# ClashLuke/LocAtE

Measured on AMD Instinct MI355X. Metric: images/sec (G+D step) 64x64 bs=64, higher is better.
Workload: dtype f32 (contractions fp32-faithful on the matrix cores: 2 x scaled fp16 operand pieces / 3 MFMAs per slice where the operand's largest magnitude comes with it, else 3 x bf16 pieces / 6 MFMAs; fp32 accumulate); 1 GPU; LocAtE G+D step, 64x64 RGB, batch 64 per GPU (the fp32 variant - the reference's own precision - of BASELINE.json configs[1]: 64x64 RGB bs 64), self/feature attention at 16x16 and 64x64, random-init weights; global_batch=64, image_size=64, parallelism=dp1, launch=hipGraph replay, G-step generator pass on a second stream

## Files before the change

include/locate_hip.h:

```cpp
#ifndef LOCATE_HIP_H
#define LOCATE_HIP_H
#include <stddef.h>
#include <stdint.h>
#ifdef __cplusplus
extern "C" {
#endif

const char* locate_last_error(void);
int locate_abi_version(void);
int locate_device_info(char* arch_name, int name_len, int* cu_count, int* wave_size);

int locate_roottanh_fwd(const float* x, float* y, int64_t n, void* absmax , void* stream);
int locate_absmax_words(void);
int locate_roottanh_bwd(const float* x, const float* gy, float* gx, int64_t n, int accumulate, void* absmax, void* stream);
int locate_absmax(const float* x, int64_t n, void* absmax, void* stream);
int locate_act_cat_rows_fwd(const float* latent, const float* pre, float* out, int rows, int z, int w, void* stream);
int locate_act_rows_bwd(const float* pre, const float* g, int64_t g_row_stride, const float* g_add, float* gpre, int rows, int w,
                        void* stream);
int locate_add3(const float* a, int64_t a_bs, const float* b, int64_t b_bs, const float* c, int64_t c_bs, float* out, int batch,
                int64_t per, void* stream);
int locate_tanh_fwd(const float* x, float* y, int64_t n, void* stream);
int locate_tanh_bwd(const float* y, const float* gy, float* gx, int64_t n, void* stream);

size_t locate_norm_stats_workspace_bytes(void);
// ... 12 lines not shown
                          void* workspace, int accumulate_dx, void* stream);
int locate_fin_norm_channels(const void* records, int n, void* stream);
size_t locate_channel_sum_workspace_bytes(int B, int C, int hw);
int locate_channel_sum(const float* g, float* out, int B, int C, int hw, int64_t batch_stride, void* workspace, void* stream);

int locate_gate_fwd(const float* x, const float* a, int a_per_plane, const float* gamma, float* out, int64_t planes, int hw,
                    void* stream);
int locate_gate_fwd_stats(const float* x, const float* a, int a_per_plane, const float* gamma, float* out, int64_t planes,
                          int hw, int groups, double* stats_partial, void* stream);
size_t locate_gate_bwd_workspace_bytes(int64_t planes);
int locate_gate_bwd_partials(int64_t planes, int hw);
int locate_gate_bwd(const float* x, const float* a, int a_per_plane, const float* gamma, const float* g, float* dx, float* da,
                    float* dgamma, int64_t planes, int hw, void* workspace, int accumulate_dx,
                    void* da_absmax , void* stream);

int locate_softmax_fwd(const float* x, float* y, int64_t rows, int n, void* stream);
int locate_softmax_bwd(const float* y, const float* gy, float* gx, int64_t rows, int n, void* stream);

int locate_upsample2x_fwd(const float* x, float* y, int64_t planes, int H, int W, void* stream);
int locate_upsample2x_bwd(const float* gy, float* gx, int64_t planes, int H, int W, void* stream);
int locate_pool2_upsample2x_fwd(const float* x, float* y, int64_t planes, int H, int W, void* stream);
int locate_pool2_upsample2x_bwd(const float* gy, float* gx, int64_t planes, int H, int W, int accumulate, void* stream);
int locate_avgpool2_fwd(const float* x, float* y, int64_t planes, int H, int W, void* stream);
int locate_avgpool2_bwd(const float* gy, float* gx, int64_t planes, int H, int W, int accumulate, void* stream);
int locate_feature_pool_fwd(const float* x, float* y, int64_t n_out, int r, void* stream);
int locate_feature_pool_bwd(const float* gy, float* gx, int64_t n_out, int r, int accumulate, void* stream);
int locate_copy_channels(const float* src, float* dst, int B, int C, int hw, int64_t src_batch_stride,
                         int64_t dst_batch_stride, int accumulate, void* stream);

size_t locate_sn_workspace_bytes(int h, int wd);
int locate_sn_power_iter(const float* w, float* u, float* v, float* sigma, float* wv, int h, int wd, void* workspace,
                         void* stream);
size_t locate_sn_table_record_bytes(void);
int locate_sn_power_iter_batched(const void* table, int n_layers, int max_h, int max_wd, void* stream);
int locate_sn_weight_bwd(const double* inner_partial, int n_partial, const float* u, const float* v, const float* sigma,
                         const float* wv, float* gw, float* du, float* dsigma_out, int h, int wd, void* stream);
size_t locate_sn_group_workspace_bytes(void);
int locate_sn_weight_bwd_grouped(const float* gy, int64_t gy_bs, const float* y, int64_t y_bs, const float* bias, int groups,
                                 int Bg, int M, int plane, const float* sigma_tab, int sigma_stride, const float* u,
                                 const float* v, const float* wv, int64_t wv_stride, float* gw, float* du,
                                 float* dsigma_total_out, int h, int wd, void* workspace, void* stream);
int locate_sn_dv_batched(const void* table, int n_layers, int max_h, int max_wd, void* stream);

size_t locate_conv_panel_bytes(const int* geom, int adjoint);
int locate_conv_pack_panel(const int* geom, int adjoint, const float* w, float* panel, void* stream);
size_t locate_conv_pack_job_bytes(void);
int locate_conv_pack_job(const int* geom, int adjoint, const float* w, float* panel, int block_start, void* job_out,
                         int* blocks_out, int direct, const void* weight_absmax);
int locate_conv_pack_panels(const void* jobs, int n_jobs, int total_blocks, int any_f16, int passes, void* stream);
int locate_conv_pack_job_is_direct(const void* job);
int locate_conv_pack_job_is_window(const void* job);
int locate_conv_win_ok(const int* geom, int adjoint_fmt, int64_t x_bs, const void* x);
size_t locate_conv_win_workspace_bytes(const int* geom, int adjoint_fmt);
size_t locate_conv_fwd_workspace_bytes(const int* geom);
size_t locate_conv_counter_bytes(void);
int locate_conv_fwd(const int* geom, const float* x, int64_t x_bs, const float* panel, const float* scale,
                    int scale_group_batch, int scale_stride, const float* bias, float* y, int64_t y_bs, void* workspace,
                    void* counters, int precision, const void* x_absmax, const void* act_epilogue, void* stream);
size_t locate_conv_dgrad_workspace_bytes(const int* geom);
int locate_conv_dgrad(const int* geom, const float* gy, int64_t gy_bs, const float* panel, const float* scale,
                      int scale_group_batch, int scale_stride, const float* bias, float* gx, int64_t gx_bs, void* workspace,
                      void* counters, int precision, const void* gy_absmax, const void* act_epilogue, void* stream);
size_t locate_conv_wgrad_workspace_bytes(const int* geom);
int locate_conv_wgrad_partials(const int* geom);
int locate_conv_wgrad(const int* geom, const float* x, int64_t x_bs, const float* gy, int64_t gy_bs, float* gw,
                      const float* w_ref, const float* inv_scale, int scale_group_batch, int scale_stride,
                      double* inner_partial, void* workspace, int precision, const void* x_absmax, const void* gy_absmax,
                      void* deferred_reduce, void* stream);
int locate_conv_wgrad_group_partials(const int* geom, int groups);
size_t locate_conv_wgrad_group_workspace_bytes(const int* geom, int groups);
size_t locate_slab_reduce_record_bytes(void);
int locate_slab_reduce_max(void);
int locate_slab_reduce_record_blocks(const void* record);
int locate_slab_reduce_batch(const void* records, int n, void* stream);

size_t locate_wgrad_batch_record_bytes(void);
int locate_wgrad_batch_max(void);
int locate_wgrad_batch_record(const int* geom, const float* x, int64_t x_bs, const float* gy, int64_t gy_bs, float* gw,
                              const float* w_ref, const float* inv_scale, int scale_group_batch, int scale_stride,
                              double* inner_partial, void* record);
int locate_wgrad_batch(const void* records, int n, void* stream);

int locate_dwconv_fwd(const int* geom, const float* x, int64_t x_bs, const float* w, const float* scale, int scale_group_batch,
                      int scale_stride, float* y, int64_t y_bs, void* stream);
int locate_dwconv_dgrad(const int* geom, const float* gy, int64_t gy_bs, const float* w, const float* scale,
                        int scale_group_batch, int scale_stride, float* gx, int64_t gx_bs, void* stream);
size_t locate_dwconv_wgrad_workspace_bytes(const int* geom);
int locate_dwconv_wgrad_partials(const int* geom);
int locate_dwconv_wgrad(const int* geom, const float* big, int64_t big_bs, const float* small, int64_t small_bs, float* gw,
                        const float* w_ref, const float* inv_scale, int scale_group_batch, int scale_stride,
                        double* inner_partial, void* workspace, void* stream);
int locate_groupdot_fwd(const float* x, int64_t x_bs, const float* w, const float* scale, int scale_group_batch,
                        int scale_stride, float* y, int B, int G, int L, void* stream);
int locate_groupdot_dgrad(const float* gy, const float* w, const float* scale, int scale_group_batch, int scale_stride,
                          float* gx, int64_t gx_bs, int B, int G, int L, void* stream);
int locate_groupdot_wgrad_partials(int G, int L);
int locate_groupdot_wgrad(const float* x, int64_t x_bs, const float* gy, float* gw, const float* w_ref, const float* inv_scale,
                          int scale_group_batch, int scale_stride, double* inner_partial, int B, int G, int L, void* stream);

size_t locate_fin_record_bytes(void);
int locate_fin_sn_dot_partials(int Bg, int M, int plane);
int locate_fin_sn_dots(const void* records, int n, void* stream);
int locate_fin_sn_rank1(const void* records, int n, void* stream);
int locate_fin_sums(const void* records, int n, void* stream);
int locate_fin_channel_slices(int B, int C, int hw);
int locate_fin_channel_sums(const void* records, int n, void* stream);
// ... 69 lines not shown
```

locate_amd/_lib.py:

```python
import ctypes
import os

import torch

_HERE = os.path.dirname(os.path.abspath(__file__))
LIB_PATH = os.path.join(_HERE, "csrc", "liblocate_hip_dbg.so" if os.environ.get("LOCATE_HIP_DEBUG_LIBRARY") == "1"
                        else "liblocate_hip.so")

c_p = ctypes.c_void_p
c_i = ctypes.c_int
c_i64 = ctypes.c_int64
c_f = ctypes.c_float
c_d = ctypes.c_double
c_sz = ctypes.c_size_t
c_ip = ctypes.POINTER(ctypes.c_int)

PROTOTYPES = {
    "locate_last_error": (ctypes.c_char_p, []),
    "locate_abi_version": (c_i, []),
    "locate_device_info": (c_i, [ctypes.c_char_p, c_i, c_ip, c_ip]),
    "locate_roottanh_fwd": (c_i, [c_p, c_p, c_i64, c_p, c_p]),
    "locate_roottanh_bwd": (c_i, [c_p, c_p, c_p, c_i64, c_i, c_p, c_p]),
    "locate_act_cat_rows_fwd": (c_i, [c_p, c_p, c_p, c_i, c_i, c_i, c_p]),
    "locate_act_rows_bwd": (c_i, [c_p, c_p, c_i64, c_p, c_p, c_i, c_i, c_p]),
    "locate_add3": (c_i, [c_p, c_i64, c_p, c_i64, c_p, c_i64, c_p, c_i, c_i64, c_p]),
    "locate_absmax_words": (c_i, []),
    "locate_wgrad_batch_record_bytes": (c_sz, []),
    "locate_wgrad_batch_max": (c_i, []),
    "locate_wgrad_batch_record": (c_i, [c_ip, c_p, c_i64, c_p, c_i64, c_p, c_p, c_p, c_i, c_i, c_p, c_p]),
    "locate_wgrad_batch": (c_i, [c_p, c_i, c_p]),
    "locate_absmax": (c_i, [c_p, c_i64, c_p, c_p]),
    "locate_tanh_fwd": (c_i, [c_p, c_p, c_i64, c_p]),
    "locate_tanh_bwd": (c_i, [c_p, c_p, c_p, c_i64, c_p]),
    "locate_norm_stats_workspace_bytes": (c_sz, []),
    "locate_norm_stats": (c_i, [c_p, c_i64, c_p, c_p, c_p]),
    "locate_norm_bwd_workspace_bytes": (c_sz, [c_i, c_i]),
    "locate_norm_fwd": (c_i, [c_p, c_p, c_i, c_p, c_p, c_i, c_p, c_i, c_i, c_i, c_i, c_p, c_p, c_p, c_p]),
    "locate_norm_bwd": (c_i, [c_p, c_p, c_p, c_p, c_i, c_p, c_i, c_p, c_p, c_p, c_i, c_i, c_i, c_i, c_p, c_i, c_p]),
    "locate_norm_bwd_fused_workspace_bytes": (c_sz, [c_i, c_i]),
    "locate_norm_bwd_fused_plane_offset": (c_sz, []),
    "locate_norm_bwd_fused": (c_i, [c_p, c_p, c_p, c_p, c_i, c_p, c_i, c_p, c_p, c_i, c_i, c_i, c_i, c_p, c_i, c_p]),
    "locate_fin_norm_channels": (c_i, [c_p, c_i, c_p]),
    "locate_channel_sum_workspace_bytes": (c_sz, [c_i, c_i, c_i]),
    "locate_channel_sum": (c_i, [c_p, c_p, c_i, c_i, c_i, c_i64, c_p, c_p]),
    "locate_gate_fwd": (c_i, [c_p, c_p, c_i, c_p, c_p, c_i64, c_i, c_p]),
    "locate_gate_fwd_stats": (c_i, [c_p, c_p, c_i, c_p, c_p, c_i64, c_i, c_i, c_p, c_p]),
    "locate_gate_bwd_workspace_bytes": (c_sz, [c_i64]),
    "locate_gate_bwd": (c_i, [c_p, c_p, c_i, c_p, c_p, c_p, c_p, c_p, c_i64, c_i, c_p, c_i, c_p, c_p]),
    "locate_softmax_fwd": (c_i, [c_p, c_p, c_i64, c_i, c_p]),
    "locate_softmax_bwd": (c_i, [c_p, c_p, c_p, c_i64, c_i, c_p]),
    "locate_upsample2x_fwd": (c_i, [c_p, c_p, c_i64, c_i, c_i, c_p]),
    "locate_upsample2x_bwd": (c_i, [c_p, c_p, c_i64, c_i, c_i, c_p]),
    "locate_pool2_upsample2x_fwd": (c_i, [c_p, c_p, c_i64, c_i, c_i, c_p]),
    "locate_pool2_upsample2x_bwd": (c_i, [c_p, c_p, c_i64, c_i, c_i, c_i, c_p]),
    "locate_avgpool2_fwd": (c_i, [c_p, c_p, c_i64, c_i, c_i, c_p]),
    "locate_avgpool2_bwd": (c_i, [c_p, c_p, c_i64, c_i, c_i, c_i, c_p]),
    "locate_feature_pool_fwd": (c_i, [c_p, c_p, c_i64, c_i, c_p]),
    "locate_feature_pool_bwd": (c_i, [c_p, c_p, c_i64, c_i, c_i, c_p]),
    "locate_copy_channels": (c_i, [c_p, c_p, c_i, c_i, c_i, c_i64, c_i64, c_i, c_p]),
    "locate_sn_workspace_bytes": (c_sz, [c_i, c_i]),
    "locate_sn_power_iter": (c_i, [c_p, c_p, c_p, c_p, c_p, c_i, c_i, c_p, c_p]),
    "locate_sn_table_record_bytes": (c_sz, []),
    "locate_sn_power_iter_batched": (c_i, [c_p, c_i, c_i, c_i, c_p]),
    "locate_sn_weight_bwd": (c_i, [c_p, c_i, c_p, c_p, c_p, c_p, c_p, c_p, c_p, c_i, c_i, c_p]),
    "locate_sn_group_workspace_bytes": (c_sz, []),
    "locate_sn_weight_bwd_grouped": (c_i, [c_p, c_i64, c_p, c_i64, c_p, c_i, c_i, c_i, c_i, c_p, c_i, c_p, c_p, c_p, c_i64, c_p,
                                           c_p, c_p, c_i, c_i, c_p, c_p]),
    "locate_sn_dv_batched": (c_i, [c_p, c_i, c_i, c_i, c_p]),
    "locate_conv_panel_bytes": (c_sz, [c_ip, c_i]),
    "locate_conv_pack_panel": (c_i, [c_ip, c_i, c_p, c_p, c_p]),
    "locate_conv_pack_job_bytes": (c_sz, []),
    "locate_conv_pack_job": (c_i, [c_ip, c_i, c_p, c_p, c_i, c_p, c_ip, c_i, c_p]),
    "locate_conv_pack_panels": (c_i, [c_p, c_i, c_i, c_i, c_i, c_p]),
    "locate_conv_pack_job_is_direct": (c_i, [c_p]),
    "locate_conv_pack_job_is_window": (c_i, [c_p]),
    "locate_conv_win_ok": (c_i, [c_ip, c_i, c_i64, c_p]),
    "locate_conv_win_workspace_bytes": (c_sz, [c_ip, c_i]),
    "locate_conv_fwd_workspace_bytes": (c_sz, [c_ip]),
    "locate_conv_counter_bytes": (c_sz, []),
    "locate_conv_fwd": (c_i, [c_ip, c_p, c_i64, c_p, c_p, c_i, c_i, c_p, c_p, c_i64, c_p, c_p, c_i, c_p, c_p, c_p]),
    "locate_conv_dgrad_workspace_bytes": (c_sz, [c_ip]),
    "locate_conv_dgrad": (c_i, [c_ip, c_p, c_i64, c_p, c_p, c_i, c_i, c_p, c_p, c_i64, c_p, c_p, c_i, c_p, c_p, c_p]),
    "locate_conv_wgrad_workspace_bytes": (c_sz, [c_ip]),
    "locate_conv_wgrad_partials": (c_i, [c_ip]),
    "locate_conv_wgrad": (c_i, [c_ip, c_p, c_i64, c_p, c_i64, c_p, c_p, c_p, c_i, c_i, c_p, c_p, c_i, c_p, c_p, c_p, c_p]),
    "locate_conv_wgrad_group_partials": (c_i, [c_ip, c_i]),
    "locate_conv_wgrad_group_workspace_bytes": (c_sz, [c_ip, c_i]),
    "locate_slab_reduce_record_bytes": (c_sz, []),
    "locate_slab_reduce_max": (c_i, []),
    "locate_slab_reduce_record_blocks": (c_i, [c_p]),
    "locate_slab_reduce_batch": (c_i, [c_p, c_i, c_p]),
    "locate_dwconv_fwd": (c_i, [c_ip, c_p, c_i64, c_p, c_p, c_i, c_i, c_p, c_i64, c_p]),
    "locate_dwconv_dgrad": (c_i, [c_ip, c_p, c_i64, c_p, c_p, c_i, c_i, c_p, c_i64, c_p]),
    "locate_dwconv_wgrad_workspace_bytes": (c_sz, [c_ip]),
    "locate_dwconv_wgrad_partials": (c_i, [c_ip]),
    "locate_dwconv_wgrad": (c_i, [c_ip, c_p, c_i64, c_p, c_i64, c_p, c_p, c_p, c_i, c_i, c_p, c_p, c_p]),
    "locate_groupdot_fwd": (c_i, [c_p, c_i64, c_p, c_p, c_i, c_i, c_p, c_i, c_i, c_i, c_p]),
    "locate_groupdot_dgrad": (c_i, [c_p, c_p, c_p, c_i, c_i, c_p, c_i64, c_i, c_i, c_i, c_p]),
    "locate_groupdot_wgrad_partials": (c_i, [c_i, c_i]),
    "locate_groupdot_wgrad": (c_i, [c_p, c_i64, c_p, c_p, c_p, c_p, c_i, c_i, c_p, c_i, c_i, c_i, c_p]),
    "locate_fin_record_bytes": (c_sz, []),
    "locate_fin_sn_dot_partials": (c_i, [c_i, c_i, c_i]),
    "locate_fin_sn_dots": (c_i, [c_p, c_i, c_p]),
    "locate_fin_sn_rank1": (c_i, [c_p, c_i, c_p]),
    "locate_fin_sums": (c_i, [c_p, c_i, c_p]),
    "locate_fin_channel_slices": (c_i, [c_i, c_i, c_i]),
    "locate_fin_channel_sums": (c_i, [c_p, c_i, c_p]),
    "locate_gate_bwd_partials": (c_i, [c_i64, c_i]),
    "locate_multi_copy_record_bytes": (c_sz, []),
    "locate_multi_copy_chunk_elems": (c_i, []),
    "locate_multi_copy": (c_i, [c_p, c_p, c_i, c_i, c_f, c_p]),
    "locate_nadam_tensor_record_bytes": (c_sz, []),
    "locate_nadam_chunk_elems": (c_i, []),
    "locate_nadam_step": (c_i, [c_p, c_p, c_p, c_i, c_i, c_d, c_d, c_d, c_d, c_d, c_d, c_p]),
    "locate_average_record_bytes": (c_sz, []),
    "locate_average_chunk_elems": (c_i, []),
    "locate_average_update": (c_i, [c_p, c_p, c_i, c_i, c_p]),
    "locate_stats_tensor_record_bytes": (c_sz, []),
    "locate_stats_record_bytes": (c_sz, []),
    "locate_stats_chunk_elems": (c_i, []),
    "locate_stats_max_blocks": (c_i, []),
    "locate_stats_workspace_bytes": (c_sz, [c_i]),
    "locate_stats_reduce": (c_i, [c_p, c_p, c_i, c_i, c_p, c_p, c_p, c_p]),
    "locate_guard_tensor_record_bytes": (c_sz, []),
    "locate_guard_verdict_bytes": (c_sz, []),
    "locate_guard_chunk_elems": (c_i, []),
    "locate_guard_max_blocks": (c_i, []),
    "locate_guard_workspace_bytes": (c_sz, [c_i]),
    "locate_guarded_nadam_step": (c_i, [c_p, c_p, c_i, c_i, c_p, c_p, c_d, c_i, c_p, c_p, c_p, c_i, c_i, c_d, c_d, c_d, c_d, c_d, c_d, c_p]),
# ... 70 lines not shown
```

locate_amd/build.py:

```python
import os
import shutil
import subprocess
import sys

CSRC = os.path.join(os.path.dirname(os.path.abspath(__file__)), "csrc")
LIB = os.path.join(CSRC, "liblocate_hip.so")
LIB_DBG = os.path.join(CSRC, "liblocate_hip_dbg.so")
DBG_SOURCES = ["conv.hip", "convwgrad.hip", "convwin.hip", "snapshot.hip"]
SOURCES = ["runtime.hip", "elementwise.hip", "norm.hip", "softmax.hip", "resample.hip", "spectral.hip", "conv.hip", "convpack.hip", "convwgrad.hip", "convwin.hip", "convfp8.hip",
           "grouped.hip", "nadam.hip", "loss.hip", "finalise.hip", "parallel.hip", "input.hip", "grid.hip", "swd.hip", "average.hip", "stats.hip", "guard.hip", "snapshot.hip"]
ARCH = "gfx950"


def _hipcc():
    for cand in (os.environ.get("HIPCC"), shutil.which("hipcc"), "/opt/rocm/bin/hipcc"):
        if cand and os.path.exists(cand):
            return cand
    raise RuntimeError("hipcc not found: the MI355X kernels cannot be built")


def _sources():
    return [s for s in SOURCES if os.path.exists(os.path.join(CSRC, s))]


def _headers():
    return [os.path.join(CSRC, h) for h in sorted(os.listdir(CSRC)) if h.endswith(".h")]


def needs_build():
    if not (os.path.exists(LIB) and os.path.exists(LIB_DBG)):
        return True
    t = min(os.path.getmtime(LIB), os.path.getmtime(LIB_DBG))
    deps = [os.path.join(CSRC, s) for s in _sources()] + _headers()
    return any(os.path.getmtime(d) > t for d in deps)


def build(force=False, verbose=True):
    if not force and not needs_build():
        return LIB
    hipcc = _hipcc()
    objs = []
    flags = ["--offload-arch=" + ARCH, "-O3", "-fPIC", "-std=c++17", "-fvisibility=hidden", "-Wall", "-Wno-unused-function",
             "-I", CSRC]
    procs = []
    hdr_time = max(os.path.getmtime(h) for h in _headers())
    for src in _sources():
        path = os.path.join(CSRC, src)
        obj = os.path.join(CSRC, src.replace(".hip", ".o"))
        objs.append(obj)
        if not force and os.path.exists(obj) and os.path.getmtime(obj) > max(os.path.getmtime(path), hdr_time):
            continue
        cmd = [hipcc] + flags + ["-c", path, "-o", obj]
        if verbose:
            print(" ".join(cmd), flush=True)
        procs.append((src, subprocess.Popen(cmd)))
    dbg_objs = list(objs)
    for src in DBG_SOURCES:
        path = os.path.join(CSRC, src)
        obj = os.path.join(CSRC, src.replace(".hip", "_dbg.o"))
        dbg_objs[dbg_objs.index(os.path.join(CSRC, src.replace(".hip", ".o")))] = obj
        if not force and os.path.exists(obj) and os.path.getmtime(obj) > max(os.path.getmtime(path), hdr_time):
            continue
# ... 19 lines not shown
```

locate_amd/csrc/conv.hip:

```cpp
#include "igemm.h"

template <int WGM, int WGN, int TM, int TN>
__global__ void __launch_bounds__(256) conv_igemm_kernel(const IgParams p) {
    constexpr int BK = IG_BK;
    constexpr int BM = WGM * TM * 32;
    constexpr int BN = WGN * TN * 32;
    constexpr int KPT = BK * BN / 256;
    constexpr int A_F4 = BK * BM / 4;
    constexpr int A_PT = (A_F4 + 255) / 256;
    static_assert(WGM * WGN == 4, "four waves");
    static_assert(BN % 64 == 0 && KPT == 8, "one 8-row group of the offset table per thread and step");
    static_assert(BK <= IG_TAIL, "panel tail shorter than the prefetch distance (one stage beyond the last)");

    __shared__ __attribute__((aligned(16))) float As[2][BK][BM];
    __shared__ __attribute__((aligned(16))) float Bs[2][BK][BN];

    int bx, by, bz;
    xcd_tile(bx, by, bz, p.tile_nphase);
    const int zphase = bz / p.ksplit, zsplit = bz - zphase * p.ksplit;
    const IgPhase& ph = p.ph[zphase];
    const int N = p.B * ph.QH * ph.QW;
    const int n0 = bx * BN;
    const int m0 = by * BM;
    if (n0 >= N) return;
// ... 641 lines not shown
}

#define IG_MAX_COUNTERS 1024
struct SplitPlan {
    int ksplit, combine, gx, gy;
    size_t slab_floats;
};

static SplitPlan igemm_split_plan(const IgParams& p, int nmax, bool have_counters) {
    SplitPlan sp;
    const int bm = igemm_bm(p.M, nmax, p.nphase);
    int min_kpad = 1 << 30;
    for (int i = 0; i < p.nphase; ++i) min_kpad = p.ph[i].Kpad < min_kpad ? p.ph[i].Kpad : min_kpad;
    int ks = igemm_ksplit(p.M, nmax, p.nphase, min_kpad);
    if (ks > min_kpad / IG_BK) ks = min_kpad / IG_BK;
    if (ks < 1) ks = 1;
    sp.ksplit = ks;
    sp.gx = (nmax + 127) / 128;
    sp.gy = (p.M + bm - 1) / bm;
    const long long ntiles = (long long)sp.gx * sp.gy * p.nphase;
    const long long tile_floats = (long long)bm * 128;
    const long long legacy = ks > 1 ? (long long)ks * p.B * p.M * p.OH * p.OW : 0;
    const long long fused = ks > 1 ? (long long)ks * ntiles * tile_floats : 0;
    sp.combine = have_counters && ks > 1 && (long long)ks * tile_floats * 4 <= (512 << 10) && ntiles <= IG_MAX_COUNTERS &&
                 fused * 4 < (1ll << 31) && (p.precision == 1 || !path_disabled("bx6")) && !path_disabled("combine");
    sp.slab_floats = (size_t)(sp.combine ? fused : legacy);
    return sp;
}

void launch_slab_reduce(const IgParams& p, hipStream_t st) {
    igemm_slab_reduce_kernel<<<stream_grid(p.slab_stride, 256), 256, 0, st>>>(p.slab, p.out, p.bias, p.scale, p.scale_bg, p.scale_stride, p.B, p.M, p.OH * p.OW,
                                                                              p.out_bs, p.slab_stride, p.ksplit, p.act_out, p.act_bs, p.mul_pre, p.mul_bs, p.out_absmax);
}

template <int NP>
static void launch_bx6(const IgParams& p, dim3 grid, int bm, bool w8, hipStream_t st) {
    if (w8) {
        if (bm == 128) conv_igemm_bx6_kernel<2, 4, 2, 1, NP, 8><<<grid, 512, 0, st>>>(p);
        else conv_igemm_bx6_kernel<2, 4, 1, 1, NP, 8><<<grid, 512, 0, st>>>(p);
        return;
    }
    with_tile<true>(bm, [&](auto t) { using T = decltype(t); conv_igemm_bx6_kernel<T::wgm, T::wgn, T::tm, T::tn, NP><<<grid, 256, 0, st>>>(p); });
}

static int launch_igemm(IgParams& p, int nmax, void* slab_ws, unsigned* counters, hipStream_t st, const char* who) {
    p.tile_nphase = (path_disabled("phasefast") || (long long)p.OH * p.OW < 1024) ? 1 : p.nphase;
    if (p.win) return launch_win_igemm(p, nmax, slab_ws, counters, st, who);
    if (skinny_ok(p)) {
        p.ksplit = 1;
        launch_skinny(p, st);
        LOCATE_LAUNCH_CHECK(who);
        return LOCATE_OK;
    }
    if (pointwise_ok(p)) {
        p.ksplit = 1;
        launch_pointwise(p, st);
        LOCATE_LAUNCH_CHECK(who);
        return LOCATE_OK;
    }
    const int bm = igemm_bm(p.M, nmax, p.nphase);
    const SplitPlan sp = igemm_split_plan(p, nmax, counters != nullptr);
    p.ksplit = sp.ksplit;
    p.combine = sp.combine;
    p.counters = counters;
    p.slab = static_cast<float*>(slab_ws);
    p.slab_stride = (long long)p.B * p.M * p.OH * p.OW;
    dim3 grid(sp.gx, sp.gy, p.nphase * p.ksplit);
    for (int i = 0; i < p.nphase; ++i)
        LOCATE_REQUIRE(round_up(p.M, bm) <= p.ph[i].ld, "%s: tile height %d does not divide the panel width %d", who, bm, p.ph[i].ld);
    if (p.precision == 3) {
        launch_fp8_igemm(p, grid, bm, st);
        LOCATE_LAUNCH_CHECK(who);
        if (p.ksplit > 1 && !p.combine) {
            LOCATE_REQUIRE(p.slab_stride < (1ll << 31), "%s: split-K output of %lld elements exceeds the 32-bit index range", who, p.slab_stride);
            launch_slab_reduce(p, st);
            LOCATE_LAUNCH_CHECK(who);
        }
        return LOCATE_OK;
    }
    const bool w8 = !path_disabled("w8") && !path_disabled("bx6") && (bm == 128 || bm == 64) &&
                    (long long)grid.x * grid.y * grid.z <= knob_int("LOCATE_W8_MAX", 320);
    if (p.precision == 2) LOCATE_REQUIRE(!path_disabled("bx6"), "%s: fp16 pieces need the bf16/fp16 MFMA kernels", who);
    if (p.precision == 1) launch_bx6<1>(p, grid, bm, w8, st);
    else if (p.precision == 2) launch_bx6<2>(p, grid, bm, w8, st);
    else if (!path_disabled("bx6")) launch_bx6<3>(p, grid, bm, w8, st);
    else with_tile<false>(bm, [&](auto t) { using T = decltype(t); conv_igemm_kernel<T::wgm, T::wgn, T::tm, T::tn><<<grid, 256, 0, st>>>(p); });
    LOCATE_LAUNCH_CHECK(who);
    if (p.ksplit > 1 && !p.combine) {
        const long long total = p.slab_stride;
        LOCATE_REQUIRE(total < (1ll << 31), "%s: split-K output of %lld elements exceeds the 32-bit index range", who, total);
        launch_slab_reduce(p, st);
        LOCATE_LAUNCH_CHECK(who);
    }
    return LOCATE_OK;
}

static size_t slab_floats(const IgParams& p, int nmax) {
    if (p.win) return win_slab_floats(p, nmax);
    if (skinny_ok(p)) return 0;
    const size_t a = igemm_split_plan(p, nmax, false).slab_floats, b = igemm_split_plan(p, nmax, true).slab_floats;
    return a > b ? a : b;
}

static void useful_taps(int in, int out, int k, int s, int pad, int* lo, int* n) {
    if (path_disabled("taps")) { *lo = 0; *n = k; return; }
    int first = -1, last = -1;
    for (int t = 0; t < k; ++t) {
        bool any = false;
        for (int o = 0; o < out && !any; ++o) {
            const int i = o * s - pad + t;
            any = i >= 0 && i < in;
        }
        if (any) { if (first < 0) first = t; last = t; }
    }
    if (first < 0) { first = 0; last = 0; }
    *lo = first; *n = last - first + 1;
}
static void useful_phase_taps(int Q, int out, int d0, int T, int* lo, int* n) {
    if (path_disabled("taps")) { *lo = 0; *n = T > 0 ? T : 1; return; }
    int first = T > 0 ? d0 - out + 1 : 0, last = d0 + Q - 1;
    if (first < 0) first = 0;
    if (last > T - 1) last = T - 1;
    if (first > last) { first = 0; last = 0; }
    *lo = first; *n = last - first + 1;
}

static void phase_taps(int parity, int pad, int K, int s, int* k0, int* d0, int* T) {
    *k0 = (parity + pad) % s;
    *d0 = (parity + pad - *k0) / s;
    *T = *k0 < K ? (K - *k0 + s - 1) / s : 0;
}

static int tap_dmin(const PackArgs& a) {
    int best = 0;
    for (int th = 0; th < a.TH; ++th)
        for (int tw = 0; tw < a.TW; ++tw) {
            const int d = (a.dy0 + a.dys * th) * a.gW + a.dx0 + a.dxs * tw;
            if (d < best) best = d;
        }
    return best;
}

static void phase_finish(IgPhase& ph, const PackArgs& pa, float* panel_base) {
    ph.wp = panel_base;
    ph.koff = reinterpret_cast<const int*>(panel_base + (size_t)pa.rows * pa.ld);
    ph.ktap = reinterpret_cast<const unsigned char*>(ph.koff + pa.rows);
    ph.w3 = reinterpret_cast<const uint4*>(panel_base + panel_split_offset(pa.rows, pa.ld) + (pa.fmt ? PANEL_HDR : 0));
    ph.a_absmax = pa.fmt ? reinterpret_cast<const unsigned*>(panel_base + panel_split_offset(pa.rows, pa.ld)) : nullptr;
    ph.w3_plane = (long long)(pa.rows / 8) * pa.ld;
    ph.dmin = pa.dmin;
    ph.K = pa.K; ph.Kpad = pa.rows - IG_TAIL; ph.ld = pa.ld;
    ph.TW = pa.TW > 0 ? pa.TW : 1; ph.tw_magic = (65536 + ph.TW - 1) / ph.TW;
// ... 115 lines not shown
        pa.s = 1;
        useful_taps(g.H, g.OH, g.KH, g.stride, g.pad_h, &pa.kh0, &pa.TH);
        useful_taps(g.W, g.OW, g.KW, g.stride, g.pad_w, &pa.kw0, &pa.TW);
        pa.K = g.C * pa.TH * pa.TW; pa.rows = round_up(pa.K, IG_KPAD) + IG_TAIL; pa.ld = round_up(g.M, 32);
        pa.gHW = g.H * g.W; pa.gW = g.W; pa.dy0 = pa.kh0 - g.pad_h; pa.dys = 1; pa.dx0 = pa.kw0 - g.pad_w; pa.dxs = 1;
        pa.dmin = tap_dmin(pa);
        pa.fmt = fmt; pa.wmax = nullptr; pa.direct = 0; pa.keep_f32 = 1;
        pa.win = 0; pa.Tp = 0; pa.urows = 0; pa.wmax_single = 0;
        batch.ph[0] = pa;
        IgPhase& ph = p.ph[0];
        phase_finish(ph, pa, panel);
        ph.T = pa.TH * pa.TW;
        ph.oy0 = ph.ox0 = 0; ph.QH = g.OH; ph.QW = g.OW;
        off = panel_floats(pa.rows, pa.ld, fmt);
        nmax = g.B * g.OH * g.OW;
    } else {
        p.B = g.B; p.C = g.M; p.H = g.OH; p.W = g.OW; p.M = g.C; p.OH = g.H; p.OW = g.W;
        p.istride = 1; p.ostep = g.stride;
        for (int py = 0; py < g.stride; ++py)
            for (int px = 0; px < g.stride; ++px) {
                int kh0, dy0, TH, kw0, dx0, TW;
                phase_taps(py, g.pad_h, g.KH, g.stride, &kh0, &dy0, &TH);
                phase_taps(px, g.pad_w, g.KW, g.stride, &kw0, &dx0, &TW);
                const int QH = py < g.H ? (g.H - py + g.stride - 1) / g.stride : 0;
                const int QW = px < g.W ? (g.W - px + g.stride - 1) / g.stride : 0;
                if (QH == 0 || QW == 0) continue;
                {
                    int lo, n;
                    useful_phase_taps(QH, g.OH, dy0, TH, &lo, &n);
                    kh0 += g.stride * lo; dy0 -= lo; TH = TH > 0 ? n : 0;
                    useful_phase_taps(QW, g.OW, dx0, TW, &lo, &n);
                    kw0 += g.stride * lo; dx0 -= lo; TW = TW > 0 ? n : 0;
                }
                IgPhase& ph = p.ph[p.nphase++];
                PackArgs pa;
                pa.w = w; pa.out = panel ? panel + off : nullptr;
                pa.M = g.M; pa.C = g.C; pa.KH = g.KH; pa.KW = g.KW; pa.mode = 1;
                pa.kh0 = kh0; pa.kw0 = kw0; pa.s = g.stride; pa.TH = TH; pa.TW = TW;
                pa.K = g.M * TH * TW; pa.rows = round_up(pa.K > 0 ? pa.K : 1, IG_KPAD) + IG_TAIL; pa.ld = round_up(g.C, 32);
                pa.gHW = g.OH * g.OW; pa.gW = g.OW; pa.dy0 = dy0; pa.dys = -1; pa.dx0 = dx0; pa.dxs = -1;
                pa.dmin = tap_dmin(pa);
                pa.fmt = fmt; pa.wmax = nullptr; pa.direct = 0; pa.keep_f32 = 1;
                pa.win = 0; pa.Tp = 0; pa.urows = 0; pa.wmax_single = 0;
                batch.ph[p.nphase - 1] = pa;
                phase_finish(ph, pa, pa.out);
                ph.T = TH * TW;
                ph.oy0 = py; ph.ox0 = px; ph.QH = QH; ph.QW = QW;
                off += panel_floats(pa.rows, pa.ld, fmt);
                const int nph = g.B * QH * QW;
                if (nph > nmax) nmax = nph;
            }
    }
    p.win = 0;
    if (adjoint_fmt & 4) {
        LOCATE_REQUIRE(win_finish(p, batch, fmt, panel, &off), "conv: this geometry has no window form (ask locate_conv_win_ok first)");
    }
    if (nmax_out) *nmax_out = nmax;
    if (panel_floats_out) *panel_floats_out = off;
    if (batch_out) *batch_out = batch;
    if (pack && p.nphase > 0)
        if (int e = launch_pack(batch, p.nphase, st, "locate_conv_pack_panel")) return e;
    return LOCATE_OK;
}

LOCATE_API size_t locate_conv_panel_bytes(const int* geom, int adjoint) {
    IgParams p;
    size_t n = 0;
    conv_plan(make_geom(geom), adjoint, nullptr, nullptr, p, nullptr, &n, false, nullptr);
    return n * sizeof(float);
}

LOCATE_API int locate_conv_pack_panel(const int* geom, int adjoint, const float* w, float* panel, void* stream) {
    const ConvGeom g = make_geom(geom);
    if (int e = geom_check(g, "locate_conv_pack_panel")) return e;
    LOCATE_REQUIRE(w && panel, "locate_conv_pack_panel: null pointer");
    IgParams p;
    return conv_plan(g, adjoint, w, panel, p, nullptr, nullptr, true, as_stream(stream));
}


LOCATE_API int locate_conv_pack_job(const int* geom, int adjoint, const float* w, float* panel, int block_start, void* job_out,
                                    int* blocks_out, int direct, const void* weight_absmax) {
    const ConvGeom g = make_geom(geom);
    if (int e = geom_check(g, "locate_conv_pack_job")) return e;
    LOCATE_REQUIRE(w && panel && job_out && blocks_out && block_start >= 0, "locate_conv_pack_job: bad arguments");
    IgParams p;
    PackBatch batch;
    if (int e = conv_plan(g, adjoint, w, panel, p, nullptr, nullptr, false, nullptr, &batch)) return e;
    LOCATE_REQUIRE(p.nphase > 0, "locate_conv_pack_job: empty panel");
    if (batch.ph[0].win) {
        for (int i = 0; i < p.nphase; ++i) {
            if (weight_absmax && (adjoint & 2)) { batch.ph[i].wmax = static_cast<const unsigned*>(weight_absmax); batch.ph[i].wmax_single = 0; }
            batch.ph[i].direct = (weight_absmax || !(adjoint & 2)) ? 1 : 0;
        }
    } else if (direct && (weight_absmax || !(adjoint & 10))) {
        const PackArgs& a0 = batch.ph[0];
        const bool transpose = a0.mode == 0 && p.nphase == 1;
        const bool adj = a0.mode == 1 && a0.KH * a0.KW <= PACK_MAX_TAPS;
        if (transpose || adj) {
            bool keep = path_disabled("bx6") || path_disabled("direct_planes_only");
            for (int i = 0; i < p.nphase; ++i) keep = keep || (p.nphase == 1 && batch.ph[i].TH * batch.ph[i].TW == 1);
            for (int i = 0; i < p.nphase; ++i) {
                batch.ph[i].wmax = static_cast<const unsigned*>(weight_absmax);
                batch.ph[i].direct = 1;
                batch.ph[i].keep_f32 = keep ? 1 : 0;
            }
        }
    }
    PackJob j = make_pack_job(batch, p.nphase);
    j.block_start = block_start;
    memcpy(job_out, &j, sizeof(PackJob));
    *blocks_out = j.gx * j.gy;
    return LOCATE_OK;
}


struct LocateActEpilogue {
    void* act_out;
    long long act_bs;
    const void* lat;
    long long lat_bs;
    int lat_z, pad;
    const void* mul_pre;
    long long mul_bs;
    void* out_absmax;
};

static int run_igemm(const ConvGeom& g, int adjoint, const float* in, int64_t in_bs, const float* panel, const float* scale,
                     int scale_bg, int scale_stride, const float* bias, float* out, int64_t out_bs, float* ws, unsigned* counters,
                     int precision, const unsigned* in_absmax, hipStream_t st, const char* who, const LocateActEpilogue* epi = nullptr) {
    const int win = (precision >> 4) & 1;
    precision &= 15;
    LOCATE_REQUIRE(precision >= 0 && precision <= 3, "%s: precision must be 0 (fp32-faithful, bf16 pieces), 1 (bf16 operands), 2 (fp32-faithful, fp16 pieces) or 3 (fp8 operands)", who);
    LOCATE_REQUIRE(precision < 2 || in_absmax, "%s: precisions 2 and 3 need the gathered tensor's absmax words", who);
    LOCATE_REQUIRE(!(win && precision == 3), "%s: no window form of the fp8 contractions", who);
    IgParams p;
    p.precision = precision;
    p.b_absmax = in_absmax;
    p.act_out = nullptr; p.act_bs = 0; p.lat = nullptr; p.lat_bs = 0; p.lat_z = 0;
    p.mul_pre = nullptr; p.mul_bs = 0; p.out_absmax = nullptr;
    int nmax = 0;
    if (int e = conv_plan(g, (adjoint & 1) | (win ? 4 : 0) | (precision == 2 ? 2 : 0) | (precision == 3 ? 8 : 0), nullptr, const_cast<float*>(panel), p, &nmax, nullptr, false, st)) return e;
    LOCATE_REQUIRE(p.nphase > 0, "%s: empty output", who);
    LOCATE_REQUIRE(!win || ((in_bs & 1) == 0 && (reinterpret_cast<uintptr_t>(in) & 7) == 0), "%s: the window form loads pixel pairs: 8-byte aligned tensor, even batch stride", who);
    p.in = in; p.out = out; p.bias = bias; p.scale = scale; p.in_bs = in_bs; p.out_bs = out_bs;
    p.scale_bg = scale_bg; p.scale_stride = scale_stride;
    {
        const long long extent = 4ll * ((long long)(p.B - 1) * in_bs + (long long)p.C * p.H * p.W);
        LOCATE_REQUIRE(in_bs >= 0 && extent > 0 && extent < (1ll << 31) - (1 << 20), "%s: gathered tensor of %lld bytes exceeds the 2 GiB a buffer descriptor addresses", who, extent);
        p.in_bytes = (unsigned)extent;
    }
    LOCATE_REQUIRE(scale_bg >= 0 && (scale_bg == 0 || g.B % scale_bg == 0), "%s: batch %d is not a multiple of the scale group %d", who, g.B, scale_bg);
    LOCATE_REQUIRE(ws || slab_floats(p, nmax) == 0, "%s: split-K needs a workspace", who);
    if (epi && epi->act_out) {
        LOCATE_REQUIRE(!epi->lat || skinny_ok(p), "%s: the latent prefix of the activated second output exists for 1x1-map layers only", who);
        LOCATE_REQUIRE(!epi->lat || (epi->lat_z > 0 && epi->act_bs >= epi->lat_z + g.M), "%s: bad latent prefix", who);
        LOCATE_REQUIRE(!epi->mul_pre, "%s: an epilogue either activates or multiplies by the activation's derivative", who);
        LOCATE_REQUIRE(epi->act_bs >= (long long)p.M * p.OH * p.OW, "%s: activated output's batch stride is smaller than one element of the batch", who);
        p.act_out = static_cast<float*>(epi->act_out); p.act_bs = epi->act_bs;
        p.lat = static_cast<const float*>(epi->lat); p.lat_bs = epi->lat_bs; p.lat_z = epi->lat ? epi->lat_z : 0;
    }
    if (epi && epi->mul_pre) {
        LOCATE_REQUIRE(epi->mul_bs >= (long long)p.M * p.OH * p.OW, "%s: pre-activation's batch stride is smaller than one element of the batch", who);
        p.mul_pre = static_cast<const float*>(epi->mul_pre); p.mul_bs = epi->mul_bs;
    }
    if (epi && (epi->act_out || epi->mul_pre)) p.out_absmax = static_cast<unsigned*>(epi->out_absmax);
    return launch_igemm(p, nmax, ws, counters, st, who);
}

static size_t igemm_ws_bytes(const int* geom, int adjoint) {
    IgParams p;
    p.precision = 0;
    int nmax = 0;
    if (conv_plan(make_geom(geom), adjoint, nullptr, nullptr, p, &nmax, nullptr, false, nullptr)) return 0;
    return (p.nphase > 0 ? slab_floats(p, nmax) : 0) * sizeof(float);
}

LOCATE_API int locate_conv_win_ok(const int* geom, int adjoint_fmt, int64_t x_bs, const void* x) {
    const ConvGeom g = make_geom(geom);
    if (geom_check(g, "locate_conv_win_ok")) return 0;
    if ((x_bs & 1) || (reinterpret_cast<uintptr_t>(x) & 7)) return 0;
    IgParams p;
    p.precision = 0;
    int nmax = 0;
    if (conv_plan(g, adjoint_fmt & 1, nullptr, nullptr, p, &nmax, nullptr, false, nullptr) || p.nphase < 1) return 0;
    p.in = static_cast<const float*>(x); p.out = nullptr; p.in_bs = x_bs; p.out_bs = 2;
    if (skinny_ok(p)) return 0;
    {
        const IgPhase& ph = p.ph[0];
        if (p.nphase == 1 && ph.T == 1 && p.istride == 1 && p.ostep == 1 && p.H == p.OH && p.W == p.OW && ph.K <= 64 && p.M <= 64 &&
            (long long)p.B * p.H * p.W >= 131072 && !path_disabled("pointwise")) return 0;
    }
    if (conv_plan(g, (adjoint_fmt & 3) | 4, nullptr, nullptr, p, &nmax, nullptr, false, nullptr) || !p.win) return 0;
    bool taps4 = p.nphase == 4;
    for (int i = 0; i < p.nphase; ++i) taps4 = taps4 && p.ph[i].T == 4;
    const bool best = p.M >= 128 && ((p.nphase == 1 && p.ph[0].T == 1 && p.C >= 384) || (taps4 && p.C >= 512));
    return best ? 1 : 2;
}
LOCATE_API size_t locate_conv_win_workspace_bytes(const int* geom, int adjoint_fmt) {
    IgParams p;
    p.precision = (adjoint_fmt & 2) ? 2 : 0;
    int nmax = 0;
    if (conv_plan(make_geom(geom), (adjoint_fmt & 3) | 4, nullptr, nullptr, p, &nmax, nullptr, false, nullptr) || !p.win) return 0;
    return win_slab_floats(p, nmax) * sizeof(float);
}

LOCATE_API size_t locate_conv_fwd_workspace_bytes(const int* geom) { return igemm_ws_bytes(geom, 0); }
LOCATE_API size_t locate_conv_dgrad_workspace_bytes(const int* geom) { return igemm_ws_bytes(geom, 1); }

LOCATE_API size_t locate_conv_counter_bytes(void) { return IG_MAX_COUNTERS * sizeof(unsigned); }

LOCATE_API int locate_conv_fwd(const int* geom, const float* x, int64_t x_bs, const float* panel, const float* scale,
                               int scale_group_batch, int scale_stride, const float* bias, float* y, int64_t y_bs,
                               void* workspace, void* counters, int precision, const void* x_absmax, const void* act_epilogue,
                               void* stream) {
    const ConvGeom g = make_geom(geom);
    if (int e = geom_check(g, "locate_conv_fwd")) return e;
    LOCATE_REQUIRE(x && panel && y, "locate_conv_fwd: null pointer");
    return run_igemm(g, 0, x, x_bs, panel, scale, scale_group_batch, scale_stride, bias, y, y_bs, static_cast<float*>(workspace),
                     static_cast<unsigned*>(counters), precision, static_cast<const unsigned*>(x_absmax), as_stream(stream), "locate_conv_fwd",
                     static_cast<const LocateActEpilogue*>(act_epilogue));
}

LOCATE_API int locate_conv_dgrad(const int* geom, const float* gy, int64_t gy_bs, const float* panel, const float* scale,
                                 int scale_group_batch, int scale_stride, const float* bias, float* gx, int64_t gx_bs,
                                 void* workspace, void* counters, int precision, const void* gy_absmax, const void* act_epilogue,
                                 void* stream) {
    const ConvGeom g = make_geom(geom);
    if (int e = geom_check(g, "locate_conv_dgrad")) return e;
    LOCATE_REQUIRE(gy && panel && gx, "locate_conv_dgrad: null pointer");
    return run_igemm(g, 1, gy, gy_bs, panel, scale, scale_group_batch, scale_stride, bias, gx, gx_bs,
                     static_cast<float*>(workspace), static_cast<unsigned*>(counters), precision, static_cast<const unsigned*>(gy_absmax),
                     as_stream(stream), "locate_conv_dgrad", static_cast<const LocateActEpilogue*>(act_epilogue));
}
// ... 1 lines not shown
```

locate_amd/csrc/igemm.h:

```cpp
#pragma once
#include "common.h"
#include <cstdlib>
#include <cstring>
#include <stdlib.h>
#include <type_traits>

#ifdef LOCATE_DEBUG_KNOBS
static bool path_disabled(const char* name) {
    static const char* env = getenv("LOCATE_DISABLE");
    return env != nullptr && strstr(env, name) != nullptr;
}
static int knob_int(const char* name, int fallback) {
    const char* v = getenv(name);
    return v != nullptr ? atoi(v) : fallback;
}
#else
static constexpr bool path_disabled(const char*) { return false; }
static constexpr int knob_int(const char*, int fallback) { return fallback; }
#endif

typedef float f32x16 __attribute__((ext_vector_type(16)));

#define IG_BK 16
#define IG_KPAD 32
#define IG_TAIL 112
#define IG_MAXT 32

struct ConvGeom {
    int B, C, H, W;
    int M, KH, KW;
    int stride, pad_h, pad_w;
    int OH, OW;
};

static int geom_check(const ConvGeom& g, const char* who) {
    LOCATE_REQUIRE(g.B > 0 && g.C > 0 && g.H > 0 && g.W > 0 && g.M > 0 && g.KH > 0 && g.KW > 0 && g.stride > 0,
                   "%s: non-positive dimension", who);
    LOCATE_REQUIRE(g.KH * g.KW <= IG_MAXT - 7, "%s: kernel %dx%d has more than %d taps", who, g.KH, g.KW, IG_MAXT - 7);
    LOCATE_REQUIRE(g.stride <= 2, "%s: stride %d unsupported (1 or 2)", who, g.stride);
    LOCATE_REQUIRE(g.OH == (g.H + 2 * g.pad_h - g.KH) / g.stride + 1 && g.OW == (g.W + 2 * g.pad_w - g.KW) / g.stride + 1,
                   "%s: output size %dx%d does not match the geometry", who, g.OH, g.OW);
    LOCATE_REQUIRE((int64_t)g.B * g.C * g.H * g.W < (1ll << 31) && (int64_t)g.B * g.M * g.OH * g.OW < (1ll << 31),
                   "%s: tensor larger than 2^31 elements", who);
    return LOCATE_OK;
}

static inline ConvGeom make_geom(const int* g) {
    ConvGeom c;
    c.B = g[0]; c.C = g[1]; c.H = g[2]; c.W = g[3]; c.M = g[4]; c.KH = g[5]; c.KW = g[6];
    c.stride = g[7]; c.pad_h = g[8]; c.pad_w = g[9]; c.OH = g[10]; c.OW = g[11];
    return c;
}

static inline int round_up(int a, int b) { return (a + b - 1) / b * b; }

static inline int pick_bm(int M) {
    const int cands[4] = {128, 96, 64, 32};
    int best = 128, best_pad = 1 << 30;
    for (int i = 0; i < 4; ++i) {
        const int pad = round_up(M, cands[i]);
        if (pad < best_pad) { best_pad = pad; best = cands[i]; }
    }
    return best;
}

template <int WGM, int WGN, int TM, int TN>
struct Tile {
    static constexpr int wgm = WGM, wgn = WGN, tm = TM, tn = TN;
};

template <bool TALL, class F>
static inline void with_tile(int bm, F&& f) {
    if constexpr (TALL) {
        if (bm == 192) return f(Tile<2, 2, 3, 2>{});
    }
    if (bm == 128) f(Tile<2, 2, 2, 2>{});
    else if (bm == 96) f(Tile<1, 4, 3, 1>{});
    else if (bm == 64) f(Tile<1, 4, 2, 1>{});
    else f(Tile<1, 4, 1, 1>{});
}

struct PackArgs {
    const float* w;
    float* out;
    int M, C, KH, KW;
    int mode;
    int kh0, kw0, s, TH, TW;
    int K, rows, ld;
    int gHW, gW, dy0, dys, dx0, dxs;
    int dmin;
    int fmt;
    const unsigned* wmax;
    int direct;
    int keep_f32;
    int win, Tp, urows, wmax_single;
};

#define PACK_MAX_TAPS 32
struct PackBatch {
    PackArgs ph[4];
};
struct PackJob {
    PackBatch batch;
    int nphase, kind;
    int gx, gy;
    int block_start, pad;
};
// ... 86 lines not shown
    h = *reinterpret_cast<unsigned*>(&hh);
    l = *reinterpret_cast<unsigned*>(&ll);
}

struct IgPhase {
    const float* wp;
    const int* koff;
    const unsigned char* ktap;
    const uint4* w3;
    const unsigned* a_absmax;
    long long w3_plane;
    int K, Kpad, ld, T;
    int dmin;
    int oy0, ox0, QH, QW;
    int TW, tw_magic;
    int dy0, dys, dx0, dxs;
    int win_Tp, win_NG, win_TR, win_NI, win_WR;
    unsigned win_wrw_mul;
    int win_wrw_s1, win_wrw_s2;
    int tapc[32] __attribute__((aligned(32)));
};

struct IgParams {
    const float* in;
    float* out;
    const float* bias;
    const float* scale;
    int scale_bg;
    int scale_stride;
    long long in_bs, out_bs;
    unsigned in_bytes;
    int B, C, H, W;
    int M, OH, OW;
    int istride, ostep, nphase;
    int ksplit;
    float* slab;
    long long slab_stride;
    int precision;
    const unsigned* b_absmax;
    float* act_out = nullptr;
    long long act_bs = 0;
    const float* lat = nullptr;
    long long lat_bs = 0;
    int lat_z = 0;
    const float* mul_pre = nullptr;
    long long mul_bs = 0;
    unsigned* out_absmax = nullptr;
    int combine;
    unsigned* counters;
    int tile_nphase;
    int win;
    int win_dbg;
    int win_U, win_slotsp, win_bm, win_bn;
    IgPhase ph[4];
};

template <int WGM, int WGN, int TM, int TN>
__device__ __forceinline__ void igemm_col_scales(const IgParams& p, const IgPhase& ph, float (&col_scale)[TN], int N, int n0,
                                                 int wn, int lane) {
    const int lcol = lane & 31;
#pragma unroll
    for (int j = 0; j < TN; ++j) {
        const int nj = n0 + (wn * TN + j) * 32 + lcol;
        const int nn = nj < N ? nj : 0;
        const int b = nn / (ph.QH * ph.QW);
        col_scale[j] = p.scale ? p.scale[(p.scale_bg ? b / p.scale_bg : 0) * p.scale_stride] : 1.0f;
    }
}

template <int WGM, int WGN, int TM, int TN>
__device__ __forceinline__ void igemm_epilogue(const IgParams& p, const IgPhase& ph, f32x16 (&acc)[TM][TN],
                                               const float (&col_scale)[TN], int N, int n0, int m0, int zsplit, int wm,
                                               int wn, int lane, float* stage, bool split) {
    const int lrow = lane >> 5, lcol = lane & 31;
    const long long plane = (long long)p.OH * p.OW;
    const int iplane = (int)plane;
    if (stage != nullptr && p.nphase == 1 && p.ostep == 1 && iplane <= 16 && (iplane & (iplane - 1)) == 0 &&
        ph.QH * ph.QW == iplane) {
        const int lp = __ffs(iplane) - 1;
        const bool fused_s = !split && (p.act_out != nullptr || p.mul_pre != nullptr);
        float am_s = 0.0f;
        float* out_base = split ? p.slab + (long long)zsplit * p.slab_stride : p.out;
        const long long obs = split ? (long long)p.M * plane : p.out_bs;
#pragma unroll
        for (int i = 0; i < TM; ++i) {
            const int mt0 = m0 + (wm * TM + i) * 32;
            float bias_v[16];
#pragma unroll
            for (int r = 0; r < 16; ++r) {
                const int m = mt0 + (r & 3) + 8 * (r >> 2) + 4 * lrow;
                const bool use = p.bias != nullptr && !split && m < p.M;
                const float* bp = use ? p.bias + m : p.in;
                bias_v[r] = use ? *bp : 0.0f;
            }
#pragma unroll
            for (int j = 0; j < TN; ++j) {
                const int nt0 = n0 + (wn * TN + j) * 32;
#pragma unroll
                for (int r = 0; r < 16; ++r) {
                    const int ml = (r & 3) + 8 * (r >> 2) + 4 * lrow;
                    stage[lcol * 33 + ml] = split ? acc[i][j][r] : fmaf(acc[i][j][r], col_scale[j], bias_v[r]);
                }
                __builtin_amdgcn_fence(__ATOMIC_SEQ_CST, "wavefront");
                const int b0 = nt0 >> lp;
                if (!fused_s) {
#pragma unroll
// ... 163 lines not shown
    g.lane_off = (unsigned)(4 * ((long long)b * p.in_bs + (long long)iy0 * p.W + ix0));
    unsigned inside = 0;
    if (n_ok) {
        for (int t = 0; t < ph.T; ++t) {
            const int th = (t * ph.tw_magic) >> 16, tw = t - th * ph.TW;
            const bool ok = (unsigned)(iy0 + ph.dy0 + ph.dys * th) < (unsigned)p.H &&
                            (unsigned)(ix0 + ph.dx0 + ph.dxs * tw) < (unsigned)p.W;
            inside |= (ok ? 1u : 0u) << t;
        }
    }
    g.outside = ~inside;
    return g;
}

__device__ __forceinline__ float gather_load(const GatherCol& g, int soff, unsigned tap) {
    const unsigned vo = ((g.outside << (31u - tap)) & 0x80000000u) | g.lane_off;
    return __builtin_bit_cast(float, __builtin_amdgcn_raw_buffer_load_b32(g.rsrc, (int)vo, soff, 0));
}

typedef int i32x8 __attribute__((ext_vector_type(8)));
typedef unsigned u32x4 __attribute__((ext_vector_type(4)));


__device__ __forceinline__ int fastdiv(int n, unsigned mul, int s1, int s2) {
    const unsigned t = __umulhi((unsigned)n, mul);
    return (int)((t + (((unsigned)n - t) >> s1)) >> s2);
}
static void fastdiv_make(unsigned d, unsigned* mul, int* s1, int* s2) {
    if (d <= 1) { *mul = 0; *s1 = 0; *s2 = 0; return; }
    int l = 0;
    while ((1ull << l) < d) ++l;
    *mul = (unsigned)(((1ull << 32) * ((1ull << l) - d)) / d + 1);
    *s1 = 1; *s2 = l - 1;
}

#define WIN_TAIL_UNITS 16

static inline int win_pick_bm(int M) { return (M >= 192 && M % 192 == 0) ? 192 : pick_bm(M); }
static inline int win_pick_bn(int bm) { return bm >= 128 ? 128 : 256; }
static inline int win_pick_sl(const int* X, int nx) {
    long long real = 0, padded = 0;
    for (int i = 0; i < nx; ++i) { real += X[i]; padded += (X[i] + 3) / 4 * 4; }
    return (padded - real) * 100 <= 15 * real ? 2 : 1;
}

static inline int win_pack_cs(int KK) { return KK <= 4 ? 64 : (KK <= 16 ? 32 : 16); }
static inline __host__ __device__ int win_pack_rg(int KK) { return KK == 1 ? 64 : 16; }
static inline size_t win_panel_floats(int urows, int ld, int fmt) { return PANEL_HDR + (size_t)(fmt ? 2 : 3) * urows * ld * 4; }

int launch_win_igemm(IgParams& p, int nmax, void* slab_ws, unsigned* counters, hipStream_t st, const char* who);
void launch_fp8_igemm(const IgParams& p, dim3 grid, int bm, hipStream_t st);
size_t win_slab_floats(const IgParams& p, int nmax);
void launch_slab_reduce(const IgParams& p, hipStream_t st);
```

Measured before the change: 7138 images/sec.

## Add scalar stencil kernel for tiny-channel adjoint convolutions

Adds a dedicated per-pixel FMA stencil kernel for adjoint convolutions with at most 4 output and 4 input channels (e.g. the RGB output layer). These cases were previously routed through the MFMA implicit-GEMM or window paths, which pad M to large tiles and waste matrix-core work and split-K slabs. The new kernel computes in plain fp32 FMA with fused bias, activation and absmax epilogues, and the planner is changed to disable the window form and keep direct panels for these geometries. The cost is a separate code path that must match the fused-epilogue semantics of the existing kernels.

Result: no change. 7153 images/sec, median of 2 (+0.2%).

```diff
diff --git a/include/locate_hip.h b/include/locate_hip.h
--- a/include/locate_hip.h
+++ b/include/locate_hip.h
@@ -88,6 +88,7 @@
 int locate_conv_pack_job_is_window(const void* job);
 int locate_conv_win_ok(const int* geom, int adjoint_fmt, int64_t x_bs, const void* x);
 size_t locate_conv_win_workspace_bytes(const int* geom, int adjoint_fmt);
+int locate_conv_stencil_ok(const int* geom);
 size_t locate_conv_fwd_workspace_bytes(const int* geom);
 size_t locate_conv_counter_bytes(void);
 int locate_conv_fwd(const int* geom, const float* x, int64_t x_bs, const float* panel, const float* scale,
diff --git a/locate_amd/_lib.py b/locate_amd/_lib.py
--- a/locate_amd/_lib.py
+++ b/locate_amd/_lib.py
@@ -75,6 +75,7 @@
     "locate_conv_pack_job_is_direct": (c_i, [c_p]),
     "locate_conv_pack_job_is_window": (c_i, [c_p]),
     "locate_conv_win_ok": (c_i, [c_ip, c_i, c_i64, c_p]),
+    "locate_conv_stencil_ok": (c_i, [c_ip]),
     "locate_conv_win_workspace_bytes": (c_sz, [c_ip, c_i]),
     "locate_conv_fwd_workspace_bytes": (c_sz, [c_ip]),
     "locate_conv_counter_bytes": (c_sz, []),
diff --git a/locate_amd/build.py b/locate_amd/build.py
--- a/locate_amd/build.py
+++ b/locate_amd/build.py
@@ -6,8 +6,8 @@
 CSRC = os.path.join(os.path.dirname(os.path.abspath(__file__)), "csrc")
 LIB = os.path.join(CSRC, "liblocate_hip.so")
 LIB_DBG = os.path.join(CSRC, "liblocate_hip_dbg.so")
-DBG_SOURCES = ["conv.hip", "convwgrad.hip", "convwin.hip", "snapshot.hip"]
-SOURCES = ["runtime.hip", "elementwise.hip", "norm.hip", "softmax.hip", "resample.hip", "spectral.hip", "conv.hip", "convpack.hip", "convwgrad.hip", "convwin.hip", "convfp8.hip",
+DBG_SOURCES = ["conv.hip", "convwgrad.hip", "convwin.hip", "convstencil.hip", "snapshot.hip"]
+SOURCES = ["runtime.hip", "elementwise.hip", "norm.hip", "softmax.hip", "resample.hip", "spectral.hip", "conv.hip", "convpack.hip", "convwgrad.hip", "convwin.hip", "convstencil.hip", "convfp8.hip",
            "grouped.hip", "nadam.hip", "loss.hip", "finalise.hip", "parallel.hip", "input.hip", "grid.hip", "swd.hip", "average.hip", "stats.hip", "guard.hip", "snapshot.hip"]
 ARCH = "gfx950"
 
diff --git a/locate_amd/csrc/conv.hip b/locate_amd/csrc/conv.hip
--- a/locate_amd/csrc/conv.hip
+++ b/locate_amd/csrc/conv.hip
@@ -717,6 +717,12 @@
         LOCATE_LAUNCH_CHECK(who);
         return LOCATE_OK;
     }
+    if (p.stencil && stencil_precision(p.precision)) {
+        p.ksplit = 1;
+        launch_stencil(p, nmax, st);
+        LOCATE_LAUNCH_CHECK(who);
+        return LOCATE_OK;
+    }
     if (pointwise_ok(p)) {
         p.ksplit = 1;
         launch_pointwise(p, st);
@@ -762,7 +768,7 @@
 
 static size_t slab_floats(const IgParams& p, int nmax) {
     if (p.win) return win_slab_floats(p, nmax);
-    if (skinny_ok(p)) return 0;
+    if (skinny_ok(p) || (p.stencil && stencil_precision(p.precision))) return 0;
     const size_t a = igemm_split_plan(p, nmax, false).slab_floats, b = igemm_split_plan(p, nmax, true).slab_floats;
     return a > b ? a : b;
 }
@@ -984,6 +990,7 @@
             }
     }
     p.win = 0;
+    p.stencil = (adjoint && stencil_ok(g)) ? 1 : 0;
     if (adjoint_fmt & 4) {
         LOCATE_REQUIRE(win_finish(p, batch, fmt, panel, &off), "conv: this geometry has no window form (ask locate_conv_win_ok first)");
     }
@@ -1032,6 +1039,7 @@
         if (transpose || adj) {
             bool keep = path_disabled("bx6") || path_disabled("direct_planes_only");
             for (int i = 0; i < p.nphase; ++i) keep = keep || (p.nphase == 1 && batch.ph[i].TH * batch.ph[i].TW == 1);
+            keep = keep || ((adjoint & 1) && stencil_ok(g));
             for (int i = 0; i < p.nphase; ++i) {
                 batch.ph[i].wmax = static_cast<const unsigned*>(weight_absmax);
                 batch.ph[i].direct = 1;
@@ -1105,6 +1113,7 @@
     p.precision = 0;
     int nmax = 0;
     if (conv_plan(make_geom(geom), adjoint, nullptr, nullptr, p, &nmax, nullptr, false, nullptr)) return 0;
+    if (p.stencil) p.precision = 1;
     return (p.nphase > 0 ? slab_floats(p, nmax) : 0) * sizeof(float);
 }
 
@@ -1112,6 +1121,7 @@
     const ConvGeom g = make_geom(geom);
     if (geom_check(g, "locate_conv_win_ok")) return 0;
     if ((x_bs & 1) || (reinterpret_cast<uintptr_t>(x) & 7)) return 0;
+    if ((adjoint_fmt & 1) && stencil_ok(g)) return 0;
     IgParams p;
     p.precision = 0;
     int nmax = 0;
diff --git a/locate_amd/csrc/convstencil.hip b/locate_amd/csrc/convstencil.hip
--- /dev/null
+++ b/locate_amd/csrc/convstencil.hip
@@ -0,0 +1,71 @@
+#include "igemm.h"
+
+#define ST_KC 16
+
+__device__ __forceinline__ void stencil_load(const GatherCol& g, const IgPhase& ph, int k0, float (&xv)[ST_KC]) {
+#pragma unroll
+    for (int i = 0; i < ST_KC; ++i) xv[i] = gather_load(g, ph.koff[k0 + i], ph.ktap[k0 + i]);
+}
+
+__global__ void __launch_bounds__(256) conv_stencil_kernel(const IgParams p) {
+    const int within = (int)blockIdx.x >> 3;
+    const int phase = within % p.nphase;
+    const int tile = (within / p.nphase) * 8 + ((int)blockIdx.x & 7);
+    const IgPhase& ph = p.ph[phase];
+    const int qhw = ph.QH * ph.QW;
+    const int N = p.B * qhw;
+    const int n = tile * 256 + (int)threadIdx.x;
+    const bool live = n < N;
+    const int nn = live ? n : 0;
+    const int b = nn / qhw, q = nn - b * qhw;
+    const int qy = q / ph.QW, qx = q - qy * ph.QW;
+    const GatherCol g = gather_setup(p, ph, n, N);
+    const float col_scale = p.scale ? p.scale[(p.scale_bg ? b / p.scale_bg : 0) * p.scale_stride] : 1.0f;
+    float acc[4] = {0.0f, 0.0f, 0.0f, 0.0f};
+    float cur[ST_KC], nxt[ST_KC];
+    stencil_load(g, ph, 0, cur);
+    for (int k0 = 0; k0 < ph.K; k0 += ST_KC) {
+        if (k0 + ST_KC < ph.K) stencil_load(g, ph, k0 + ST_KC, nxt);
+#pragma unroll
+        for (int i = 0; i < ST_KC; ++i) {
+            const float* __restrict__ wr = ph.wp + (long long)(k0 + i) * ph.ld;
+#pragma unroll
+            for (int m = 0; m < 4; ++m) acc[m] = fmaf(wr[m], cur[i], acc[m]);
+        }
+#pragma unroll
+        for (int i = 0; i < ST_KC; ++i) cur[i] = nxt[i];
+    }
+    const long long plane = (long long)p.OH * p.OW;
+    const long long pix = (long long)(ph.oy0 + qy * p.ostep) * p.OW + (ph.ox0 + qx * p.ostep);
+    const bool fused = p.act_out != nullptr || p.mul_pre != nullptr;
+    float am = 0.0f;
+#pragma unroll
+    for (int m = 0; m < 4; ++m) {
+        if (m < p.M && live) {
+            const long long rel = (long long)m * plane + pix;
+            float v = fmaf(acc[m], col_scale, p.bias ? p.bias[m] : 0.0f);
+            if (p.mul_pre != nullptr) {
+                v = roottanh_grad_f(p.mul_pre[(long long)b * p.mul_bs + rel], v);
+                am = fmaxf(am, fabsf(v));
+            }
+            p.out[(long long)b * p.out_bs + rel] = v;
+            if (p.mul_pre == nullptr && p.act_out != nullptr) {
+                const float a = roottanh_f(v);
+                p.act_out[(long long)b * p.act_bs + rel] = a;
+                am = fmaxf(am, fabsf(a));
+            }
+        }
+    }
+    if (fused && p.out_absmax != nullptr) absmax_publish_wave(am, p.out_absmax);
+}
+
+void launch_stencil(const IgParams& p, int nmax, hipStream_t st) {
+    const int tiles = round_up((nmax + 255) / 256, 8);
+    conv_stencil_kernel<<<tiles * p.nphase, 256, 0, st>>>(p);
+}
+
+LOCATE_API int locate_conv_stencil_ok(const int* geom) {
+    const ConvGeom g = make_geom(geom);
+    if (geom_check(g, "locate_conv_stencil_ok")) return 0;
+    return stencil_ok(g) ? 1 : 0;
+}
diff --git a/locate_amd/csrc/igemm.h b/locate_amd/csrc/igemm.h
--- a/locate_amd/csrc/igemm.h
+++ b/locate_amd/csrc/igemm.h
@@ -53,6 +53,11 @@
 }
 
 static inline int round_up(int a, int b) { return (a + b - 1) / b * b; }
+
+static bool stencil_ok(const ConvGeom& g) {
+    return !path_disabled("stencil") && g.M <= 4 && g.C <= 4 && g.C * g.KH * g.KW <= 128;
+}
+static inline bool stencil_precision(int precision) { return precision == 0 || precision == 2; }
 
 static inline int pick_bm(int M) {
     const int cands[4] = {128, 96, 64, 32};
@@ -245,6 +250,7 @@
     int win;
     int win_dbg;
     int win_U, win_slotsp, win_bm, win_bn;
+    int stencil;
     IgPhase ph[4];
 };
 
@@ -514,3 +520,5 @@
 void launch_fp8_igemm(const IgParams& p, dim3 grid, int bm, hipStream_t st);
 size_t win_slab_floats(const IgParams& p, int nmax);
 void launch_slab_reduce(const IgParams& p, hipStream_t st);
+
+void launch_stencil(const IgParams& p, int nmax, hipStream_t st);
```
